# s3prl/s3prl

Measured on AMD Instinct MI355X. Metric: encoder-frames/sec (20 ms stride) HuBERT-base 32x10 s @16 kHz, higher is better.
Workload: dtype f32; 1 GPU; hubert_base random-init, 32x10 s @16 kHz per GPU, one UpstreamExpert.forward per step: all 13 hidden_states (fp32) written; utterances_per_gpu=32, global_batch=32, samples=160000, frames_per_utt=499, parallelism=dp1, lengths=equal, gather=none

## Files before the change

### s3prl_amd/csrc/engine.hip

```cpp
#include "engine_internal.h"

namespace s3e {

thread_local std::string g_err;

long conv_len(const s3enc_config& c, long n, int upto ) {
    for (int i = 0; i < upto; ++i) n = n >= c.conv_kernel[i] ? (n - c.conv_kernel[i]) / c.conv_stride[i] + 1 : 0;
    return n;
}

int valid_frames(const s3enc_config& c, long length, long n_max) {
    const long T = conv_len(c, n_max, c.n_conv);
    if (T <= 0) return 0;
    long v;
    if (c.family == S3ENC_WAV2VEC2 || c.family == S3ENC_DISTILLER || c.family == S3ENC_WAV2VEC) {
        v = conv_len(c, length, c.n_conv);
    } else {
        const long chunk = n_max / T;
        v = (length + chunk - 1) / chunk;
    }
    if (v > T) v = T;
    if (v < 0) v = 0;
    return (int)v;
}
// ... 236 lines not shown
            }
            if (e->x3 || (e->x2_conv_f32_from && i >= e->x2_conv_f32_from)) UP(upload_x3(e->conv[i].w3, t2, C, (long)k * cin));
            if (e->dtype == F32 && !e->x3 && k == 3 && c.conv_stride[i] == 2) {
                std::vector<float> wp((size_t)C * cin);
                for (int co = 0; co < C; ++co)
                    for (int ci = 0; ci < cin; ++ci) wp[(size_t)co * cin + ci] = t2[(long)co * 3 * cin + ci] + t2[(long)co * 3 * cin + 2 * cin + ci];
                UP(upload_f32(e->conv[i].wp, wp));
            }
        }
        if (c.conv_bias) {
            GET(p + ".0.bias", C, t);
            UP(upload_f32(e->conv[i].bias, t));
            e->conv[i].has_bias = true;
        }
        if (c.extractor_layer_norm) {
            GET(p + ".2.1.weight", C, t);
            UP(upload_f32(e->conv[i].lng, t));
            GET(p + ".2.1.bias", C, t);
            UP(upload_f32(e->conv[i].lnb, t));
        } else if (i == 0) {
            GET(p + ".2.weight", C, t);
            UP(upload_f32(e->gn_g, t));
            GET(p + ".2.bias", C, t);
            UP(upload_f32(e->gn_b, t));
        }
    }
    if (!c.no_feature_layer_norm) {
        GET("layer_norm.weight", C, t);
        UP(upload_f32(e->fln_g, t));
        GET("layer_norm.bias", C, t);
        UP(upload_f32(e->fln_b, t));
    }
    GET("post_extract_proj.weight", (long)D * C, t);
    UP(upload_gemm_w(e->proj_w, t, D, C, e->dtype, e->x2));
    e->x2_proj_f32 = e->x2 && !c.no_feature_layer_norm && c.family != S3ENC_DISTILLER && x3_shape_ok(D, C, C);
    if (e->x3 || e->x2_proj_f32) UP(upload_x3(e->proj_w3, t, D, C));
    GET("post_extract_proj.bias", D, t);
    UP(upload_f32(e->proj_b, t));

    const bool conf = c.layer_type == 1;
    if (conf) {
    } else if (c.pos_conv_depth > 1) {
        const int G = c.conv_pos_groups, Dg = D / G;
        int k = c.conv_pos / c.pos_conv_depth;
        k = k < 3 ? 3 : k;
        const bool k16 = e->dtype != F32 || e->x3;
        int kp = k;
        if (k16)
            while ((kp & 1) || ((long)kp * Dg) % 128) ++kp;
        e->pos_k = kp;
        e->pos_pad = k / 2;
        e->pos_ws.resize(c.pos_conv_depth);
        e->pos_bs.resize(c.pos_conv_depth);
        for (int i = 0; i < c.pos_conv_depth; ++i) {
            const std::string p = "encoder.pos_conv." + std::to_string(i) + ".0";
            std::vector<float> w, wp((size_t)D * Dg * kp, 0.f);
            GET(p + ".weight", (long)D * Dg * k, w);
            for (long r = 0; r < (long)D * Dg; ++r)
                for (int j = 0; j < k; ++j) wp[r * kp + j] = w[r * k + j];
            if (e->x3) {
                UP(upload_posconv_x3(e->pos_ws[i], wp, D, G, kp));
            } else {
                pack_posconv(wp, D, G, kp, e->dtype, t2);
                UP(upload_cvt(e->pos_ws[i], t2, e->dtype));
            }
            GET(p + ".bias", D, t);
            UP(upload_f32(e->pos_bs[i], t));
        }
        UP(upload_f32(e->ones, std::vector<float>(D, 1.f)));
        UP(upload_f32(e->zeros, std::vector<float>(D, 0.f)));
    } else {
        const int K = c.conv_pos, G = c.conv_pos_groups, Dg = D / G;
        std::vector<float> g, v;
        GET(enc0 + ".pos_conv.0.weight_g", K, g);
        GET(enc0 + ".pos_conv.0.weight_v", (long)D * Dg * K, v);
        std::vector<double> nrm(K, 0.0);
        for (long i = 0; i < (long)D * Dg; ++i)
            for (int k = 0; k < K; ++k) nrm[k] += (double)v[i * K + k] * v[i * K + k];
        for (int k = 0; k < K; ++k) nrm[k] = (double)g[k] / std::sqrt(nrm[k]);
        for (long i = 0; i < (long)D * Dg; ++i)
            for (int k = 0; k < K; ++k) v[i * K + k] = (float)(v[i * K + k] * nrm[k]);
        int kp = K;
        if (e->dtype != F32 || e->x3)
            while ((kp & 1) || ((long)kp * Dg) % 128) ++kp;
        e->pos_k = kp;
        e->pos_pad = K / 2;
        if (kp != K) {
            std::vector<float> vp((size_t)D * Dg * kp, 0.f);
            for (long r = 0; r < (long)D * Dg; ++r)
                for (int j = 0; j < K; ++j) vp[r * kp + j] = v[r * K + j];
            v.swap(vp);
        }
        pack_posconv(v, D, G, kp, e->dtype, t2);
        UP(upload_cvt(e->pos_w, t2, e->dtype));
        if (e->x3) UP(upload_posconv_x3(e->pos_w3, v, D, G, kp));
        GET(enc0 + ".pos_conv.0.bias", D, t);
        UP(upload_f32(e->pos_b, t));
    }
    if (!multires) {
        GET("encoder.layer_norm.weight", D, t);
        UP(upload_f32(e->eln_g, t));
        GET("encoder.layer_norm.bias", D, t);
        UP(upload_f32(e->eln_b, t));
    }

    const float qscale = (1.0f / std::sqrt((float)(D / H))) * (e->dtype != F32 ? 1.44269504088896340736f : 1.0f);
    e->x2_attn_f32 = e->x2 && !multires && x3_shape_ok(D, D, D);
    auto load_layer = [&](const std::string& p, LayerW& L) -> int {
        std::vector<float> w(3L * D * D), bb(3L * D);
        const char* names[3] = {"q_proj", "k_proj", "v_proj"};
        for (int s = 0; s < 3; ++s) {
            GET(p + ".self_attn." + names[s] + ".weight", (long)D * D, t);
            GET(p + ".self_attn." + names[s] + ".bias", D, t2);
            const float sc = s == 0 ? qscale : 1.f;
            for (long i = 0; i < (long)D * D; ++i) w[(long)s * D * D + i] = t[i] * sc;
            for (int i = 0; i < D; ++i) bb[(long)s * D + i] = t2[i] * sc;
        }
        UPW(L.wqkv, w, 3L * D, D, 2);
        if (e->x3) UP(upload_x3(L.wqkv3, w, 3L * D, D));
        UP(upload_f32(L.bqkv, bb));
        GET(p + ".self_attn.out_proj.weight", (long)D * D, t);
        UP(upload_gemm_w(L.wo, t, D, D, e->dtype, e->x2));
        if (e->x3 || e->x2_attn_f32) UP(upload_x3(L.wo3, t, D, D));
        GET(p + ".self_attn.out_proj.bias", D, t);
        UP(upload_f32(L.bo, t));
        GET(p + ".self_attn_layer_norm.weight", D, t);
        UP(upload_f32(L.ln1g, t));
        GET(p + ".self_attn_layer_norm.bias", D, t);
        UP(upload_f32(L.ln1b, t));
        GET(p + ".fc1.weight", (long)F * D, t);
        UPW(L.w1, t, F, D, 4);
        if (e->x3) UP(upload_x3(L.w13, t, F, D));
        GET(p + ".fc1.bias", F, t);
        UP(upload_f32(L.b1, t));
        GET(p + ".fc2.weight", (long)D * F, t);
        UPW(L.w2, t, D, F, 8);
        if (e->x3) UP(upload_x3(L.w23, t, D, F));
        GET(p + ".fc2.bias", D, t);
        UP(upload_f32(L.b2, t));
        GET(p + ".final_layer_norm.weight", D, t);
        UP(upload_f32(L.ln2g, t));
        GET(p + ".final_layer_norm.bias", D, t);
        UP(upload_f32(L.ln2b, t));
        if (c.rel_pos && c.gru_rel_pos) {
            GET(p + ".self_attn.grep_linear.weight", 8 * 64, t);
            UP(upload_f32(L.grep_w, t));
            GET(p + ".self_attn.grep_linear.bias", 8, t);
            UP(upload_f32(L.grep_b, t));
// ... 798 lines not shown
        e->taps["feat_ln"] = {featT, M * C, proj32 ? (int)F32 : dt};
        if (dbg_stop == 20) return 0;
    }
    const int si_proj = (dist || (conf && c.layer_norm_first)) ? 0 : -1;
    float* xproj = sink.slot32(si_proj) ? sink.slot32(si_proj) : (float*)x32;
    {
        GemmParams g{};
        g.A = featT;
        g.lda = C;
        g.a_bs = T * C;
        g.W = e->proj_w.p;
        g.W_x3 = e->proj_w3.p;
        g.bias = (const float*)e->proj_b.p;
        g.M = (int)T;
        g.N = D;
        g.K = C;
        g.batches = B;
        g.row_limit = d_valid;
        g.out32 = xproj;
        g.out16 = sink.slot16(si_proj);
        g.ldo = D;
        g.o_bs = T * D;
        {
            Prof pr(e, st, "gemm:proj", 2.0 * M * D * C, ((double)M * C + (double)D * C) * es + (double)M * D * 4);
            if (proj32 && dt != F32) {
                if (!gemm_x3_eligible(g)) return fail("post_extract_proj is not a shape of the three-term GEMM (internal)");
                HIP_TRY(launch_gemm(F32, g, st));
            } else {
                HIP_TRY(launch_gemm(dt, wsplit_of(e, g), st));
            }
        }
        e->taps["proj"] = {xproj, M * D, F32};
        if (dbg_stop == 21) return 0;
        HIP_TRY(sink.emit(si_proj, xproj, false));
        HIP_TRY(sink.done(si_proj));
    }
    if (mr) {
        std::vector<const int*> dv(plan.blocks.size(), d_valid);
        for (size_t bi = 1; bi < plan.blocks.size(); ++bi) dv[bi] = (const int*)(d_tbl + (size_t)B * 20) + (bi - 1) * (size_t)B;
        return multires_tail(e, st, B, plan, dv, xproj, out, (long)layer_stride, fo) ? 1 : 0;
    }
    if (conf) {
        ConformerBufs cb{x32, xpc, xT, qkv, attn, tmp1, tmp2, hbuf, cbuf, pbuf};
        return conformer_tail(e, st, sink, B, T, d_valid, xproj, cb);
    }
    float* x_cur;
    void* a16_cur = nullptr;
    {
        const int si0 = si_hidden(0);
        float* pc_out = prel ? (sink.slot32(si0) ? sink.slot32(si0) : other(xproj)) : other(xproj);
        PosConvParams p{};
        p.x = xproj;
        p.w = e->pos_w.p;
        p.bias = (const float*)e->pos_b.p;
        p.out = pc_out;
        p.B = B;
        p.T = (int)T;
        p.D = D;
        p.G = c.conv_pos_groups;
        p.K = e->pos_k;
        p.pad = e->pos_pad;
        auto run_conv = [&](PosConvParams& q) -> hipError_t {
            if (e->x3) return launch_posconv16(3, q, st);
            return dt == F32 ? launch_posconv(q, st) : launch_posconv16(dt, q, st);
        };
        if (c.pos_conv_depth > 1) {
            const float* cur_in = xproj;
            const int gelu_act = (dt != F32 || e->x3) ? 2 : 1;
            for (int i = 0; i < c.pos_conv_depth; ++i) {
                p.x = cur_in;
                p.w = e->pos_ws[i].p;
                p.bias = (const float*)e->pos_bs[i].p;
                p.out = (float*)tmp1;
                p.K = e->pos_k;
                p.pad = e->pos_pad;
                p.plain = 1;
                {
                    Prof pr(e, st, "posconv", 2.0 * M * D * (D / p.G) * (2 * e->pos_pad + 1), (double)M * D * 8);
                    HIP_TRY(run_conv(p));
                }
                Prof pr(e, st, "layernorm:posconv", 0, (double)M * D * 8);
                HIP_TRY(launch_layernorm(F32, (const float*)tmp1, (const float*)e->ones.p, (const float*)e->zeros.p, M, D, gelu_act,
                                         (float*)tmp2, nullptr, st));
                cur_in = (const float*)tmp2;
            }
            Prof pr(e, st, "residual_add", 0, (double)M * D * 12);
            HIP_TRY(launch_add(xproj, (const float*)tmp2, pc_out, M * D, st));
            p.out = pc_out;
        } else {
            Prof pr(e, st, "posconv", 2.0 * M * D * (D / p.G) * c.conv_pos, (double)M * D * 8 + (double)D * (D / p.G) * c.conv_pos * 4);
            if (e->x3) p.w = e->pos_w3.p;
            HIP_TRY(run_conv(p));
        }
        e->taps["posconv"] = {p.out, M * D, F32};
        if (dbg_stop == 22) return 0;
        if (prel) {
            x_cur = pc_out;
            if (sink.mode == 1) HIP_TRY(sink.emit(si0, pc_out));
            HIP_TRY(sink.done(si0));
        } else {
            float* h0 = sink.slot32(si0) ? sink.slot32(si0) : other(pc_out);
            void* h16 = dt == F32 ? nullptr : (sink.slot16(si0) ? sink.slot16(si0) : xT);
            Prof pr(e, st, "layernorm:enc", 0, (double)M * D * (8 + (dt == F32 ? 0 : es)));
            LnGate g0;
            if (gated) {
                g0.gw = (const float*)e->layers[0].grep_w.p;
                g0.gb = (const float*)e->layers[0].grep_b.p;
                g0.ga = (const float*)e->layers[0].grep_a.p;
                g0.gate = (float*)gate;
                g0.T = (int)T;
                g0.H = H;
            }
            HIP_TRY(launch_layernorm(dt, pc_out, (const float*)e->eln_g.p, (const float*)e->eln_b.p, M, D, 0, h0, h16, st,
                                     sink.acc(si0, 2), g0));
            x_cur = h0;
            a16_cur = h16;
            HIP_TRY(sink.done(si0));
        }
    }
    const float* d_table = c.rel_pos ? (const float*)e->rel_table.p : nullptr;
    auto gate_of = [&](int l) {
        LnGate g;
        if (gated && l < NL) {
            const LayerW& w = e->layers[l];
// ... 403 lines not shown
```

### s3prl_amd/csrc/engine_internal.h

```cpp
#pragma once
#include <hip/hip_runtime.h>

#include <algorithm>
#include <cmath>
#include <cstdio>
#include <cstring>
#include <map>
#include <memory>
#include <mutex>
#include <string>
#include <thread>
#include <vector>

#include "../../include/s3enc.h"
#include "kernels.h"

namespace s3e {
using namespace s3;


extern thread_local std::string g_err;

inline int fail(const std::string& msg) {
    g_err = msg;
// ... 98 lines not shown

inline hipError_t upload_f32(DevBuf& d, const std::vector<float>& v) {
    hipError_t e = d.ensure(v.size() * 4 + 16);
    if (e != hipSuccess) return e;
    return hipMemcpy(d.p, v.data(), v.size() * 4, hipMemcpyHostToDevice);
}
template <typename F>
inline void parallel_ranges(long n, long min_per_thread, F&& fn) {
    unsigned nt = std::thread::hardware_concurrency();
    nt = nt < 1 ? 1 : (nt > 16 ? 16 : nt);
    if ((long)nt > n / std::max<long>(1, min_per_thread)) nt = (unsigned)std::max<long>(1, n / std::max<long>(1, min_per_thread));
    if (nt <= 1) {
        fn(0L, n);
        return;
    }
    std::vector<std::thread> th;
    unsigned started = 0;
    try {
        th.reserve(nt);
        for (; started < nt; ++started) th.emplace_back([&fn, n, nt, started]() { fn(n * started / nt, n * (started + 1) / nt); });
    } catch (...) {
    }
    for (unsigned t = started; t < nt; ++t) fn(n * t / nt, n * (t + 1) / nt);
    for (auto& x : th) x.join();
}

inline hipError_t upload_cvt(DevBuf& d, const std::vector<float>& v, int dtype) {
    if (dtype == F32) return upload_f32(d, v);
    std::vector<uint16_t> h(v.size());
    const float* src = v.data();
    uint16_t* dst = h.data();
    if (dtype == BF16)
        parallel_ranges((long)v.size(), 1 << 20, [=](long a, long b) { for (long i = a; i < b; ++i) dst[i] = h_bf16(src[i]); });
    else
        parallel_ranges((long)v.size(), 1 << 20, [=](long a, long b) { for (long i = a; i < b; ++i) dst[i] = h_f16(src[i]); });
    hipError_t e = d.ensure(h.size() * 2 + 16);
    if (e != hipSuccess) return e;
    return hipMemcpy(d.p, h.data(), h.size() * 2, hipMemcpyHostToDevice);
}

inline void pack_posconv(const std::vector<float>& w, int D, int G, int K, int dtype, std::vector<float>& out) {
    const int Dg = D / G;
    out.assign((size_t)G * K * Dg * Dg, 0.f);
    for (int gi = 0; gi < G; ++gi)
        for (int n = 0; n < Dg; ++n)
            for (int ci = 0; ci < Dg; ++ci)
                for (int k = 0; k < K; ++k) {
                    const float x = w[((long)(gi * Dg + n) * Dg + ci) * K + k];
                    if (dtype == F32)
                        out[((((long)gi * K + k) * (Dg / 16) + ci / 16) * Dg + n) * 16 + ((((ci % 16) >> 2) ^ pc_w_swizzle(n)) << 2) + (ci & 3)] = x;
                    else
                        out[(((long)gi * Dg + n) * K + k) * Dg + ci] = x;
                }
}

inline hipError_t upload_f16_hi_lo(DevBuf& d, const std::vector<float>& v, long N, long K) {
    std::vector<uint16_t> h((size_t)N * 2 * K);
    const float* src = v.data();
    uint16_t* dst = h.data();
    parallel_ranges(N, std::max<long>(1, (1 << 19) / std::max<long>(1, K)), [=](long n0, long n1) {
        for (long n = n0; n < n1; ++n)
            for (long k = 0; k < K; ++k) {
                const float w = src[(size_t)n * K + k];
                const uint16_t hi = h_f16(w);
                dst[(size_t)n * 2 * K + k] = hi;
                dst[(size_t)n * 2 * K + K + k] = h_f16(w - h_from16(hi, F16));
            }
    });
    hipError_t e = d.ensure(h.size() * 2 + 16);
    if (e != hipSuccess) return e;
    return hipMemcpy(d.p, h.data(), h.size() * 2, hipMemcpyHostToDevice);
}
inline hipError_t upload_gemm_w(DevBuf& d, const std::vector<float>& v, long N, long K, int dtype, bool x2) {
    return x2 ? upload_f16_hi_lo(d, v, N, K) : upload_cvt(d, v, dtype);
}

inline unsigned mx_e2m1(float x) {
    const unsigned sign = x < 0.f ? 8u : 0u;
    const float a = x < 0.f ? -x : x;
    unsigned c;
    if (a < 0.25f) c = 0; else if (a == 0.25f) c = 0;
    else if (a < 0.75f) c = 1; else if (a == 0.75f) c = 2;
    else if (a < 1.25f) c = 2; else if (a == 1.25f) c = 2;
    else if (a < 1.75f) c = 3; else if (a == 1.75f) c = 4;
    else if (a < 2.5f) c = 4; else if (a == 2.5f) c = 4;
    else if (a < 3.5f) c = 5; else if (a == 3.5f) c = 6;
    else if (a < 5.f) c = 6; else if (a == 5.f) c = 6;
    else c = 7;
    return sign | c;
}
inline void pack_mx4_lo_rows(const float* w, long K, long n0, long n1, uint8_t* data, uint8_t* scales) {
    const long kb = K / 32;
    for (long n = n0; n < n1; ++n)
        for (long b = 0; b < kb; ++b) {
            float lo[32], amax = 0.f;
            for (int i = 0; i < 32; ++i) {
                const float x = w[(size_t)n * K + b * 32 + i];
                lo[i] = x - h_from16(h_f16(x), F16);
                const float a = lo[i] < 0.f ? -lo[i] : lo[i];
                amax = a > amax ? a : amax;
            }
            int ex = -127;
            if (!(amax <= 3.0e38f)) {
                ex = 128;
            } else if (amax > 0.f) {
                ex = (int)ceilf(log2f(amax / 6.f));
// ... 70 lines not shown
struct ConvW {
    DevBuf w, bias, lng, lnb;
    DevBuf w3;
    DevBuf wp;
    bool has_bias = false;
};

struct BlockW {
    std::vector<LayerW> layers;
    DevBuf eln_g, eln_b;
};
struct AdapterConvW {
    DevBuf w, w3;
    DevBuf g, b;
};
struct AdapterW {
    AdapterConvW up, down;
    int kind = 0;
    int up_rate = 1, down_rate = 1;
};

struct W2vW {
    std::vector<DevBuf> ext_w, ext_g, ext_b;
    std::vector<DevBuf> agg_w, agg_bias, agg_g, agg_b;
    std::vector<DevBuf> vq_w, vq_b;
    std::vector<DevBuf> km_w;
    DevBuf km_g, km_b, emb_t;
    DevBuf table;
};

struct ProfRec {
    int kind;
    hipEvent_t a, b;
};

}

using namespace s3e;

struct s3enc_encoder {
    s3enc_config cfg;
    int device = 0;
    int dtype = F32;
    bool x3 = false;
    bool x2 = false;
    int x2_conv_f32_from = 0;
    bool x2_proj_f32 = false;
    bool x2_attn_f32 = false;
    int es = 4;
    std::vector<ConvW> conv;
    DevBuf gn_g, gn_b;
    DevBuf fln_g, fln_b, proj_w, proj_b, pos_w, pos_b, eln_g, eln_b;
    DevBuf proj_w3, pos_w3;
    std::vector<LayerW> layers;
    std::vector<ConformerLayerW> cf_layers;
    DevBuf rope_tab, pe_tab;
    int rope_T = 0, pe_T = 0;
    DevBuf rel_table;
    int rel_R = 0;
    std::vector<DevBuf> pos_ws, pos_bs;
    int pos_k = 0, pos_pad = 0;
    DevBuf ones, zeros;
    DevBuf head_w1, head_b1, head_w2, head_b2, head_w13, head_w23;
    DevBuf wsum_part;
    std::vector<BlockW> mr_blocks;
    std::vector<AdapterW> mr_adapters;
    DevBuf ws_mr;
    std::unique_ptr<W2vW> w2v;
    s3enc_wav2vec_config w2v_cfg = {};
    float* aux_codewords = nullptr;
    long long* aux_codeids = nullptr;

    std::map<const void*, std::unique_ptr<MxImage>> mx_images;

    Tuning tun;
    bool has_tuning = false;

    DevBuf ws;
    DevBuf small;
    void* pinned = nullptr;
    static constexpr int RING = 4;
    size_t slot_bytes = 0;
    hipEvent_t slot_ev[RING] = {};
    int slot_next = 0;

    std::vector<hipEvent_t> layer_events;

    static constexpr int STATUS_RING = 8;
    DevBuf status_dev;
    int* status_host = nullptr;
    hipEvent_t status_ev[STATUS_RING] = {};
    bool status_busy[STATUS_RING] = {};
    int status_next = 0;
    int status_sticky = 0;
    int status_collect(bool wait) {
        int running = 0;
        for (int k = 0; k < STATUS_RING; ++k) {
            const int i = (status_next + k) % STATUS_RING;
            if (!status_busy[i]) continue;
            const hipError_t q = wait ? hipEventSynchronize(status_ev[i]) : hipEventQuery(status_ev[i]);
            if (q == hipErrorNotReady) {
                (void)hipGetLastError();
                ++running;
                continue;
            }
            status_busy[i] = false;
            if (q == hipSuccess) status_sticky |= ((volatile int*)status_host)[i];
        }
        return running;
    }

    int prof = 0;
    std::vector<std::string> kinds;
// ... 153 lines not shown
```

### s3prl_amd/csrc/kernels.h

```cpp
#pragma once
#include <cstring>
#include <vector>

#include "common.h"

namespace s3 {
int device_cus();

template <auto Kern>
inline hipError_t ensure_dynamic_lds(int bytes) {
    static int granted[64] = {};
    int dev = 0;
    hipError_t e = hipGetDevice(&dev);
    if (e != hipSuccess) return e;
    if (dev >= 0 && dev < 64 && granted[dev] >= bytes) return hipSuccess;
    e = hipFuncSetAttribute((const void*)Kern, hipFuncAttributeMaxDynamicSharedMemorySize, bytes);
    if (e == hipSuccess && dev >= 0 && dev < 64) granted[dev] = bytes;
    return e;
}

struct Tuning {
    int gemm_variant = 3;
    int gemm_lds_pad = 0;
    int gemm32_big = 1;
    int gemm_x3_tile = 1;
    int gemm16_big = 3;
    int gemm16_pp = 0;
    int gemm16_mx = 14;
    int reserve_cus = 0;
    int gemm16_rows = 1;
    int attn_lds_pad = 0;
    int attn_persist = 0;
    int conv0_nt = 1;
    int conv_f22 = 1;
    int conv0_fast = 1;
    int ws_inplace = 1;
    int gelu32 = 1;
    int x3_pack_cache = 0;
    int fp16x2_conv1_f32 = 0;
    int ln_rows = 1;
    int ln_preload = 1;
    int ln1_fold = 1;
    int gn_lag_one_block = 1;
    int forward_chain = 1;
    int comm_self_p2p = 0;
};
extern Tuning g_tuning;
extern thread_local const Tuning* t_tuning;
inline const Tuning& tuning() { return t_tuning ? *t_tuning : g_tuning; }
struct TuningScope {
    const Tuning* prev;
    explicit TuningScope(const Tuning* t) : prev(t_tuning) { if (t) t_tuning = t; }
    ~TuningScope() { t_tuning = prev; }
};
int tuning_set(Tuning& t, const char* key, int value, const char** err);

extern thread_local int* t_status;
struct StatusScope {
    int* prev;
    explicit StatusScope(int* p) : prev(t_status) { t_status = p; }
    ~StatusScope() { t_status = prev; }
};

struct GemmParams {
    const void* A;
    long lda, a_bs;
    const void* W;
    const void* W_x3 = nullptr;
    const float* bias;
    int M, N, K, batches;
    int act;
    const float* residual;
    const int* row_limit;
    const float2* res_ln_stats = nullptr;
    const float* res_ln_g = nullptr;
    const float* res_ln_b = nullptr;
    float* out32;
    void* out16;
    long ldo, o_bs;
    int variant = -1;
    long ldw = 0;
    int wsplit = 0;
    const void* W4 = nullptr;
    const void* W4s = nullptr;
    int mxw = 0;
};
bool gemm16_mx_eligible(int dtype, const GemmParams& p);
// ... 59 lines not shown
    float w = 0.f;
    int mode = 0;
    int norm = 0;
    int init = 0;
};
struct LnGate {
    const float* gw = nullptr;
    const float* gb = nullptr;
    const float* ga = nullptr;
    float* gate = nullptr;
    int T = 0, H = 0;
};
hipError_t launch_layernorm(int dtype, const float* x, const float* gamma, const float* beta, long rows, int C, int act,
                            float* out32, void* out16, hipStream_t s, const LnAcc& fa = LnAcc(), const LnGate& gt = LnGate(),
                            float2* stats_out = nullptr);
hipError_t launch_emit_state(int dtype, const float* x, long rows, int C, void* out16, const LnAcc& fa, hipStream_t s);
hipError_t launch_add(const float* a, const float* b, float* out, long n, hipStream_t s);

struct AttnParams {
    const void* qkv;
    void* out;
    const int* valid;
    int B, T, H;
    const float* bias_table;
    int table_R = 0;
    const float* gate;
    int out_f32 = 0;
    int probe = 0;
    const float* rel_P = nullptr;
    const float* rel_qadd = nullptr;
};
hipError_t launch_attention(int dtype, const AttnParams& p, hipStream_t s);
hipError_t launch_wavlm_gate(const float* x, const float* grep_w , const float* grep_b ,
                             const float* grep_a , int B, int T, int H, float* gate, hipStream_t s);

struct ConformerConvParams {
    const float* x;
    const float* taps;
    const float* shift;
    float* out;
    int B, T, D, K;
};
hipError_t launch_conformer_conv(const ConformerConvParams& p, hipStream_t s);
hipError_t launch_rope(const float* x, const float* table, long rows, int T, int D, float* out, hipStream_t s);

struct PosConvParams {
    const float* x;
    const void* w;
    const float* bias;
    float* out;
    int B, T, D, G, K;
    int pad = -1;
    int plain = 0;
};
hipError_t launch_posconv(const PosConvParams& p, hipStream_t s);
__host__ __device__ inline int pc_w_swizzle(int co) { return ((co & 15) >> 3) << 1; }
hipError_t launch_posconv16(int dtype, const PosConvParams& p, hipStream_t s);

struct PadCopyParams {
    const float* a;
    long a_bs;
    const float* b;
    long b_bs;
    int B, rows, D;
    int lead, total;
    const int* zero_from;
    float* out32;
    void* out16;
};
hipError_t launch_pad_copy(int dtype, const PadCopyParams& p, hipStream_t s);
constexpr int GS_BLOCKS = 64;
hipError_t launch_group1_stats(const float* x, long bs, long count, int B, double* partial , hipStream_t s);
struct AdapterApplyParams {
    const float* conv;
    long conv_bs;
    const double* partial;
    double count;
    const float* gamma;
    const float* beta;
    const float* r1;
    long r1_bs;
    int r1_mul, r1_div;
    const float* r2;
    long r2_bs;
    int r2_mul, r2_div;
    float scale;
    int B, rows, D;
    int lead, total;
    const int* zero_from;
    float* out32;
    void* out16;
    int fast_gelu;
};
hipError_t launch_adapter_apply(int dtype, const AdapterApplyParams& p, hipStream_t s);
hipError_t launch_emit_upsampled(int dtype, const float* x, long x_bs, int factor, int B, int rows_out, int D, float* out32,
                                 void* out16, hipStream_t s);

hipError_t launch_emit_upsampled_acc(const float* x, long x_bs, int factor, int B, int rows_out, int D, const LnAcc& fa,
                                     hipStream_t s);

struct Gn1ApplyParams {
    const float* x;
    long x_bs;
    const double* partial;
    double count;
    const float* gamma;
// ... 50 lines not shown
```

### s3prl_amd/csrc/multires.hip

```cpp
#include "engine_internal.h"

namespace s3e {

long mr_adapter_frames(int k, long T, int up, int down, int kind) {
    long n = T;
    if (kind != 1) n = std::min<long>((long)up * T + k - 1, (long)up * T);
    if (kind != 2) {
        const long ld = (n + 2 * ((k - 1) / 2) - k) / down + 1;
        const long n2 = std::min(ld, (n + down - 1) / down);
        n = kind == 0 ? std::min(n2, ((long)up * T + down - 1) / down) : n2;
    }
    return n;
}

void mr_plan(const s3enc_config& c, long T0, MrPlan& plan) {
    const int R = c.mr_pairs + 1, k = c.mr_kernel;
    long ds[S3ENC_MAX_RES], lcm = 1;
    ds[0] = 1;
    for (int i = 0; i < c.n_conv; ++i) ds[0] *= c.conv_stride[i];
    for (int i = 0; i < R - 1; ++i) ds[i + 1] = ds[i] * c.mr_ratios[2 * i + 1] / c.mr_ratios[2 * i];
    for (int i = 0; i < R; ++i) {
        long a = lcm, b = ds[i];
        while (b) {
            const long r = a % b;
// ... 80 lines not shown
        attn = wb.take((size_t)Mc * D * es);
        hbuf = wb.take((size_t)Mc * F * es);
        for (int i = 0; i < R - 1; ++i) res[i] = (float*)wb.take((size_t)B * plan.blocks[i].T * D * 4);
        for (int i = 0; i < 2; ++i) {
            pad32[i] = (float*)wb.take((size_t)B * Pc * D * 4);
            if (dt != F32) pad16[i] = wb.take((size_t)B * Pc * D * 2);
        }
        convout = (float*)wb.take((size_t)B * Lc * D * 4);
        gpart = (double*)wb.take((size_t)B * GS_BLOCKS * 2 * 8);
        if (!pass) HIP_TRY(e->ws_mr.ensure_on_stream(wb.off + 4096, st));
    }

    int si = 0;
    bool first_term = true;
    auto emit = [&](const float* x, long T, int factor) -> int {
        if (fo.featurize) {
            if (fo.w[si] != 0.f) {
                LnAcc fa;
                fa.acc = (float*)out;
                fa.w = fo.w[si];
                fa.mode = 1;
                fa.norm = fo.feat_norm;
                fa.init = first_term;
                first_term = false;
                Prof pr(e, st, "emit_state", 0, (double)B * plan.T_out * D * (4.0 / factor + 8));
                HIP_TRY(launch_emit_upsampled_acc(x, T * D, factor, B, (int)plan.T_out, D, fa, st));
            }
            ++si;
            return 0;
        }
        float* o32 = out16 ? nullptr : (float*)out + (long)si * layer_stride;
        void* o16 = out16 ? (void*)((u16*)out + (long)si * layer_stride) : nullptr;
        {
            Prof pr(e, st, "emit_state", 0, (double)B * plan.T_out * D * (4.0 / factor + (out16 ? 2 : 4)));
            HIP_TRY(launch_emit_upsampled(out16 ? dt : (int)F32, x, T * D, factor, B, (int)plan.T_out, D, o32, o16, st));
        }
        if (si < (int)e->layer_events.size()) HIP_TRY(hipEventRecord(e->layer_events[si], st));
        ++si;
        return 0;
    };

    auto run_block = [&](int bi, float* x, float* y_out) -> int {
        BlockW& bw = e->mr_blocks[bi];
        const MrBlockPlan& bp = plan.blocks[bi];
        const long T = bp.T, M = (long)B * T;
        const double gM = (double)M;
        const int NLb = (int)bw.layers.size();
        float* cur = x;
        auto pick = [&](const float* busy) { return busy == hA ? hB : hA; };
        if (bi == 0) {
            PosConvParams p{};
            p.x = x;
            p.w = e->x3 ? e->pos_w3.p : e->pos_w.p;
            p.bias = (const float*)e->pos_b.p;
            p.out = hA;
            p.B = B;
            p.T = (int)T;
            p.D = D;
            p.G = c.conv_pos_groups;
            p.K = e->pos_k;
            p.pad = e->pos_pad;
            Prof pr(e, st, "posconv", 2.0 * gM * D * (D / p.G) * c.conv_pos, gM * D * 8 + (double)D * (D / p.G) * p.K * 4);
            HIP_TRY(e->x3 ? launch_posconv16(3, p, st) : (dt == F32 ? launch_posconv(p, st) : launch_posconv16(dt, p, st)));
            cur = hA;
        }
        if (!prel) {
            float* h0 = pick(cur);
            Prof pr(e, st, "layernorm:enc", 0, gM * D * (8 + (dt == F32 ? 0 : es)));
            HIP_TRY(launch_layernorm(dt, cur, (const float*)bw.eln_g.p, (const float*)bw.eln_b.p, M, D, 0, h0,
                                     dt == F32 ? nullptr : xT, st));
            cur = h0;
        }
        if (emit(cur, T, bp.factor)) return 1;
        for (int l = 0; l < NLb; ++l) {
            LayerW& Lw = bw.layers[l];
            const bool lastl = l == NLb - 1;
            const void* a_in;
            if (prel) {
                Prof pr(e, st, "layernorm:ln1", 0, gM * D * (4 + es));
                HIP_TRY(launch_layernorm(dt, cur, (const float*)Lw.ln1g.p, (const float*)Lw.ln1b.p, M, D, 0,
                                         dt == F32 ? (float*)xT : nullptr, dt == F32 ? nullptr : xT, st));
                a_in = xT;
            } else {
                a_in = dt == F32 ? (const void*)cur : (const void*)xT;
            }
            {
                GemmParams g{};
                g.A = a_in;
                g.lda = D;
                g.W = Lw.wqkv.p;
                g.W_x3 = Lw.wqkv3.p;
                g.bias = (const float*)Lw.bqkv.p;
                g.M = (int)M;
                g.N = 3 * D;
                g.K = D;
                g.batches = 1;
                g.ldo = 3 * D;
                if (dt == F32) g.out32 = (float*)qkv; else g.out16 = qkv;
                Prof pr(e, st, "gemm:qkv", 2.0 * gM * 3 * D * D, (gM * D + 3.0 * D * D + gM * 3 * D) * es);
                HIP_TRY(launch_gemm(dt, wsplit_of(e, g), st));
            }
            {
                AttnParams a{};
                a.qkv = qkv;
                a.out = attn;
                a.valid = d_valid[bi];
// ... 250 lines not shown
```

### s3prl_amd/csrc/ops.hip

```cpp
#include "engine_internal.h"

namespace s3 {
Tuning g_tuning;
thread_local const Tuning* t_tuning = nullptr;
thread_local int* t_status = nullptr;

int tuning_set(Tuning& t, const char* key, int value, const char** err) {
    struct Key {
        const char* name;
        int Tuning::*field;
        int lo, hi;
    };
    static const Key keys[] = {
        {"gemm_variant", &Tuning::gemm_variant, 0, 63},      {"gemm_lds_pad", &Tuning::gemm_lds_pad, 0, 120 * 1024},
        {"gemm32_big", &Tuning::gemm32_big, 0, 5},           {"gemm_x3_tile", &Tuning::gemm_x3_tile, 0, 5},
        {"gemm16_big", &Tuning::gemm16_big, 0, 10},          {"gemm16_rows", &Tuning::gemm16_rows, 0, 1},
        {"attn_lds_pad", &Tuning::attn_lds_pad, 0, 48 * 1024}, {"conv0_nt", &Tuning::conv0_nt, 0, 1},
        {"ws_inplace", &Tuning::ws_inplace, 0, 1},           {"gemm16_pp", &Tuning::gemm16_pp, 0, 3},
        {"gemm16_mx", &Tuning::gemm16_mx, 0, 31},            {"reserve_cus", &Tuning::reserve_cus, 0, 128},
        {"x3_pack_cache", &Tuning::x3_pack_cache, 0, 1},     {"gelu32", &Tuning::gelu32, 0, 1},
        {"comm_self_p2p", &Tuning::comm_self_p2p, 0, 1},     {"attn_persist", &Tuning::attn_persist, 0, 1},
        {"fp16x2_conv1_f32", &Tuning::fp16x2_conv1_f32, 0, 1}, {"gn_lag_one_block", &Tuning::gn_lag_one_block, 0, 1},
        {"ln_rows", &Tuning::ln_rows, 1, 2},                 {"ln1_fold", &Tuning::ln1_fold, 0, 1},
        {"ln_preload", &Tuning::ln_preload, 0, 1},           {"forward_chain", &Tuning::forward_chain, 0, 1},
        {"conv0_fast", &Tuning::conv0_fast, 0, 1},           {"conv_f22", &Tuning::conv_f22, 0, 1},
    };
    static thread_local char msg[160];
    if (!key) {
        *err = "s3enc_set_tuning: null key";
        return 1;
    }
    for (const Key& k : keys)
        if (!strcmp(key, k.name)) {
            if (value < k.lo || value > k.hi) {
                snprintf(msg, sizeof(msg), "%s must be %d..%d", k.name, k.lo, k.hi);
                *err = msg;
                return 1;
            }
            t.*(k.field) = value;
            return 0;
        }
    snprintf(msg, sizeof(msg), "s3enc_set_tuning: unknown key '%s'", key);
    *err = msg;
    return 1;
}
}

extern "C" {

int s3enc_set_tuning(const char* key, int32_t value) {
    const char* err = nullptr;
    if (tuning_set(g_tuning, key, value, &err)) return fail(err);
    return 0;
}
int s3enc_set_handle_tuning(s3enc_handle h, const char* key, int32_t value) {
    if (!h) return fail("null handle");
    if (!h->has_tuning) {
        h->tun = g_tuning;
        h->has_tuning = true;
    }
    const char* err = nullptr;
    if (tuning_set(h->tun, key, value, &err)) return fail(err);
    return 0;
}

int s3enc_op_gemm(int32_t dtype, const void* A, int64_t lda, int64_t a_batch_stride, const void* W, const float* bias, int32_t M,
                  int32_t N, int32_t K, int32_t batches, int32_t act, const float* residual, const int32_t* row_limit,
                  float* out32, void* out16, int64_t ldo, int64_t o_batch_stride, void* stream) {
    GemmParams g{};
    g.A = A;
    g.lda = lda;
    g.a_bs = a_batch_stride;
    g.W = W;
    g.bias = bias;
    g.M = M;
    g.N = N;
    g.K = K;
    g.batches = batches;
// ... 239 lines not shown
    hipStream_t st = (hipStream_t)stream;
    const size_t tbl = (size_t)B * 16, part = stats_partial_elems(B, nm);
    DevBuf buf;
    Bump sz(nullptr);
    sz.take(tbl);
    sz.take((size_t)B * sizeof(float2));
    sz.take((size_t)B * C * sizeof(float2));
    sz.take(part * 8);
    HIP_TRY(buf.ensure(sz.off + 256));
    Bump bb(buf.p);
    char* d_tbl = (char*)bb.take(tbl);
    float2* d_norm = (float2*)bb.take((size_t)B * sizeof(float2));
    float2* d_gn = (float2*)bb.take((size_t)B * C * sizeof(float2));
    double* d_part = (double*)bb.take(part * 8);
    std::vector<char> host(tbl);
    memcpy(host.data(), wavs, (size_t)B * 8);
    for (int b = 0; b < B; ++b) ((long*)(host.data() + (size_t)B * 8))[b] = (long)lengths[b];
    HIP_TRY(hipMemcpy(d_tbl, host.data(), tbl, hipMemcpyHostToDevice));
    WavTable wt{(const float* const*)d_tbl, (const long*)(d_tbl + (size_t)B * 8), B, nm};
    HIP_TRY(launch_wav_norm_stats(wt, normalize, d_part, d_norm, st));
    if (gn_gamma) HIP_TRY(launch_gn_stats(wt, d_norm, w0, gn_gamma, gn_beta, C, k0, stride, L0, d_part, nullptr, d_gn, st));
    Conv0Params p{};
    p.wav = wt;
    p.norm = d_norm;
    p.w0 = w0;
    p.bias = bias;
    p.gn = gn_gamma ? d_gn : nullptr;
    p.ln_g = ln_gamma;
    p.ln_b = ln_beta;
    p.C = C;
    p.k0 = k0;
    p.s0 = stride;
    p.L0 = L0;
    p.out = out;
    HIP_TRY(launch_conv0(dtype, p, st));
    HIP_TRY(hipStreamSynchronize(st));
    return 0;
}

int s3enc_op_wavlm_gate(const float* x, const float* grep_w, const float* grep_b, const float* grep_a, int32_t B, int32_t T,
                        int32_t H, float* gate, void* stream) {
    if (!x || !grep_w || !grep_b || !grep_a || !gate) return fail("s3enc_op_wavlm_gate: null argument");
    if (B <= 0 || T <= 0 || H <= 0) return fail("s3enc_op_wavlm_gate: bad shape");
    HIP_TRY(launch_wavlm_gate(x, grep_w, grep_b, grep_a, B, T, H, gate, (hipStream_t)stream));
    return 0;
}

int s3enc_op_posconv(int32_t dtype, const float* x, const float* w_host, const float* bias, int32_t B, int32_t T, int32_t D,
                     int32_t G, int32_t K, float* out, void* stream) {
    if (!x || !w_host || !bias || !out) return fail("s3enc_op_posconv: null argument");
    if (G <= 0 || D % G) return fail("s3enc_op_posconv: D must be a multiple of groups");
    const int Dg = D / G;
    std::vector<float> w(w_host, w_host + (size_t)D * Dg * K), packed;
    DevBuf dw;
    if (dtype == 3) {
        HIP_TRY(upload_posconv_x3(dw, w, D, G, K));
    } else {
        pack_posconv(w, D, G, K, dtype, packed);
        HIP_TRY(upload_cvt(dw, packed, dtype));
    }
    PosConvParams p{};
    p.x = x;
    p.w = dw.p;
    p.bias = bias;
    p.out = out;
    p.B = B;
    p.T = T;
    p.D = D;
    p.G = G;
    p.K = K;
    HIP_TRY(dtype == F32 ? launch_posconv(p, (hipStream_t)stream) : launch_posconv16(dtype, p, (hipStream_t)stream));
    HIP_TRY(hipStreamSynchronize((hipStream_t)stream));
    return 0;
}

int s3enc_weighted_sum(const float* hs, int64_t layer_stride, int32_t L, const float* w, int32_t normalize, int64_t rows, int32_t D,
                       float* out, void* stream) {
    if (!hs || !w || !out) return fail("s3enc_weighted_sum: null argument");
    if (L <= 0 || L > S3_WS_MAX_LAYERS) return fail("s3enc_weighted_sum: 1..32 layers");
    if (D <= 0 || (D & 3) || D > 2048) return fail("s3enc_weighted_sum: D must be a multiple of 4, <= 2048");
    HIP_TRY(launch_weighted_sum(hs, layer_stride, L, w, normalize, rows, D, out, (hipStream_t)stream));
    return 0;
}

int64_t s3enc_weighted_sum_backward_scratch(int64_t rows, int32_t L) {
    return rows > 0 && L > 0 ? (int64_t)weighted_sum_bwd_blocks(rows) * L : 0;
}

int s3enc_weighted_sum_backward(const float* hs, int64_t layer_stride, int32_t L, int32_t normalize, int64_t rows, int32_t D,
                                const float* grad_out, float* grad_w, double* scratch, void* stream) {
    if (!hs || !grad_out || !grad_w || !scratch) return fail("s3enc_weighted_sum_backward: null argument");
    if (L <= 0 || L > S3_WS_MAX_LAYERS) return fail("s3enc_weighted_sum_backward: 1..32 layers");
    if (D <= 0 || (D & 3) || D > 2048) return fail("s3enc_weighted_sum_backward: D must be a multiple of 4, <= 2048");
    if (rows <= 0) return fail("s3enc_weighted_sum_backward: no rows");
    HIP_TRY(launch_weighted_sum_bwd(hs, layer_stride, L, normalize, rows, D, grad_out, scratch, grad_w, (hipStream_t)stream));
    return 0;
}

static FbankParams fbank_params(const s3enc_fbank_config* c) {
    FbankParams f;
    f.sample_rate = c->sample_rate;
    f.num_mel_bins = c->num_mel_bins;
    f.frame_length_ms = c->frame_length_ms;
    f.frame_shift_ms = c->frame_shift_ms;
    f.preemph = c->preemphasis;
    f.delta_order = c->delta_order;
    f.delta_win = c->delta_win_length;
    f.use_cmvn = c->use_cmvn;
    f.cmvn_eps = c->cmvn_eps;
    return f;
}

int s3enc_fbank_num_frames(const s3enc_fbank_config* cfg, int64_t n_samples, int32_t* frames) {
    if (!cfg || !frames) return fail("s3enc_fbank_num_frames: null argument");
    *frames = (int32_t)fbank_num_frames(n_samples, fbank_params(cfg));
    return 0;
// ... 25 lines not shown
```

### s3prl_amd/csrc/posconv.hip

```cpp
#include "kernels.h"

namespace s3 {
namespace {

constexpr int PC_TM = 128;
constexpr int PC_FT = 2;

struct PcWork {
    int b, g, tile;
    bool live;
};
__device__ __forceinline__ PcWork pc_work(const PosConvParams& p, int ntiles) {
    PcWork w;
    const int wg = blockIdx.x;
    if (p.G & 7) {
        w.tile = wg % ntiles;
        const int r = wg / ntiles;
        w.g = r % p.G;
        w.b = r / p.G;
        w.live = w.b < p.B;
        return w;
    }
    const int per = ntiles * p.B, xcd = wg & 7, local = wg >> 3;
    w.g = xcd + 8 * (local / per);
// ... 61 lines not shown

    const float* xrow = xs + (wave * (16 * PC_FT) + l15) * RS + 4 * kk;
    for (int j = 0; j < K; ++j) {
        if (j + 1 < K) wload(j + 1);
        const float* wb = wl + (j & 1) * WSZ + l15 * 16 + 4 * (kk ^ pc_w_swizzle(l15));
        const float* xa = xrow + j * RS;
#pragma unroll
        for (int cc = 0; cc < NCC; ++cc) {
            float4 a[PC_FT];
#pragma unroll
            for (int f = 0; f < PC_FT; ++f) a[f] = *(const float4*)(xa + f * 16 * RS + 16 * cc);
#pragma unroll
            for (int n = 0; n < NT; ++n) {
                const float4 w = *(const float4*)(wb + (cc * DG + n * 16) * 16);
#pragma unroll
                for (int f = 0; f < PC_FT; ++f) {
                    acc[f][n] = __builtin_amdgcn_mfma_f32_16x16x4f32(a[f].x, w.x, acc[f][n], 0, 0, 0);
                    acc[f][n] = __builtin_amdgcn_mfma_f32_16x16x4f32(a[f].y, w.y, acc[f][n], 0, 0, 0);
                    acc[f][n] = __builtin_amdgcn_mfma_f32_16x16x4f32(a[f].z, w.z, acc[f][n], 0, 0, 0);
                    acc[f][n] = __builtin_amdgcn_mfma_f32_16x16x4f32(a[f].w, w.w, acc[f][n], 0, 0, 0);
                }
            }
        }
        if (j + 1 < K) wstore((j + 1) & 1);
        __syncthreads();
    }

#pragma unroll
    for (int f = 0; f < PC_FT; ++f)
#pragma unroll
        for (int n = 0; n < NT; ++n) {
            const int c = g * DG + n * 16 + l15;
            const float bias = p.bias[c];
#pragma unroll
            for (int r = 0; r < 4; ++r) {
                const int t = t0 + wave * (16 * PC_FT) + 16 * f + 4 * kk + r;
                if (t < p.T) {
                    const long o = ((long)b * p.T + t) * p.D + c;
                    p.out[o] = p.plain ? acc[f][n][r] + bias : p.x[o] + gelu_erf(acc[f][n][r] + bias);
                }
            }
        }
}

template <int DG>
hipError_t pc_launch(const PosConvParams& p, hipStream_t s) {
    const int rows = PC_TM + p.K - 1;
    const size_t lds = (size_t)(((rows * (DG + 8) + 3) & ~3) + 2 * DG * DG) * sizeof(float);
    hipError_t e = ensure_dynamic_lds<posconv_kernel<DG>>((int)lds);
    if (e != hipSuccess) return e;
    dim3 grid((unsigned)(((p.T + PC_TM - 1) / PC_TM) * p.G * p.B));
    hipLaunchKernelGGL(posconv_kernel<DG>, grid, dim3(256), lds, s, p);
    return hipGetLastError();
}


constexpr int P16_TM = 256;
constexpr int P16_KC = 128;

template <typename T> struct Mma16x16;
template <> struct Mma16x16<bf16_tag> {
    static __device__ __forceinline__ f32x4 run(const uint4& a, const uint4& b, const f32x4& c) {
        return __builtin_amdgcn_mfma_f32_16x16x32_bf16(__builtin_bit_cast(bf16x8, a), __builtin_bit_cast(bf16x8, b), c, 0, 0, 0);
    }
};
template <> struct Mma16x16<f16_tag> {
    static __device__ __forceinline__ f32x4 run(const uint4& a, const uint4& b, const f32x4& c) {
        return __builtin_amdgcn_mfma_f32_16x16x32_f16(__builtin_bit_cast(f16x8, a), __builtin_bit_cast(f16x8, b), c, 0, 0, 0);
    }
};

template <typename T, int DG, bool X3>
__global__ __launch_bounds__(256) void posconv16_kernel(PosConvParams p) {
    constexpr int NT = DG / 16;
    constexpr int CH = DG / 8;
    constexpr int NLW = DG * 16 / 256;
    constexpr int WBUF = DG * 256;
    constexpr int NS = X3 ? 2 : 1;
    constexpr int TMF = X3 ? 128 : P16_TM;
    constexpr int MT = TMF / 64;
    extern __shared__ __attribute__((aligned(16))) char lds16[];
    const int K = p.K;
    const int ROWS = (TMF + K - 1 + 15) & ~15;
    const size_t WIN = (size_t)CH * ROWS * 16;
    char* win = lds16;
    char* wl = lds16 + NS * WIN;

    const PcWork wk = pc_work(p, (p.T + TMF - 1) / TMF);
    if (!wk.live) return;
    const int b = wk.b, g = wk.g;
    const int t0 = wk.tile * TMF;
    const int tid = threadIdx.x, lane = tid & 63, wave = tid >> 6;
    const int l15 = lane & 15, kgrp = lane >> 4;
    const int pad = p.pad >= 0 ? p.pad : K / 2;
    const long Ktot = (long)K * DG;

    const char* wg = (const char*)p.w + (long)g * DG * Ktot * 2;
    const long plane_bytes = (long)p.G * DG * Ktot * 2;
    u32x4 wreg[NS][NLW];
#define P16_WLOAD(kc_)                                                                                        \
    _Pragma("unroll") for (int s_ = 0; s_ < NS; ++s_) _Pragma("unroll") for (int i_ = 0; i_ < NLW; ++i_) {  \
        const int e_ = tid + 256 * i_, n_ = e_ >> 4, c_ = e_ & 15;                                          \
        wreg[s_][i_] = *(const u32x4*)(wg + s_ * plane_bytes + ((long)n_ * Ktot + (long)(kc_) * P16_KC + c_ * 8) * 2); \
    }
#define P16_WSTORE(buf_)                                                                                      \
    _Pragma("unroll") for (int s_ = 0; s_ < NS; ++s_) _Pragma("unroll") for (int i_ = 0; i_ < NLW; ++i_) {  \
// ... 74 lines not shown
#pragma unroll
        for (int m = 0; m < MT; ++m)
#pragma unroll
            for (int r = 0; r < 4; ++r) {
                const int t = t0 + wave * (TMF / 4) + m * 16 + 4 * kgrp + r;
                if (t < p.T) {
                    const long o = ((long)b * p.T + t) * p.D + c;
                    const float y = acc[m][n][r] + bias;
                    p.out[o] = p.plain ? y : p.x[o] + gelu_fast(y);
                }
            }
    }
}

template <typename T, int DG, bool X3>
hipError_t pc16_launch(const PosConvParams& p, hipStream_t s) {
    constexpr int NS = X3 ? 2 : 1, TMF = X3 ? 128 : P16_TM;
    const int ROWS = (TMF + p.K - 1 + 15) & ~15;
    const size_t lds = (size_t)NS * (DG / 8) * ROWS * 16 + (size_t)NS * 2 * DG * 256;
    if (lds > 160 * 1024) return hipErrorInvalidValue;
    hipError_t e = ensure_dynamic_lds<posconv16_kernel<T, DG, X3>>((int)lds);
    if (e != hipSuccess) return e;
    dim3 grid((unsigned)(((p.T + TMF - 1) / TMF) * p.G * p.B));
    hipLaunchKernelGGL((posconv16_kernel<T, DG, X3>), grid, dim3(256), lds, s, p);
    return hipGetLastError();
}

template <typename T, bool X3 = false>
hipError_t pc16_dispatch(const PosConvParams& p, int dg, hipStream_t s) {
    switch (dg) {
        case 32: return pc16_launch<T, 32, X3>(p, s);
        case 48: return pc16_launch<T, 48, X3>(p, s);
        case 64: return pc16_launch<T, 64, X3>(p, s);
    }
    return hipErrorInvalidValue;
}

}

hipError_t launch_posconv16(int dtype, const PosConvParams& p, hipStream_t s) {
    if (p.B <= 0 || p.T <= 0) return hipSuccess;
    const int dg = p.D / p.G;
    if (dg * p.G != p.D || (p.K & 1) || ((long)p.K * dg) % P16_KC) return hipErrorInvalidValue;
    if (dtype == BF16) return pc16_dispatch<bf16_tag>(p, dg, s);
    if (dtype == F16) return pc16_dispatch<f16_tag>(p, dg, s);
    if (dtype == 3) return pc16_dispatch<bf16_tag, true>(p, dg, s);
    return hipErrorInvalidValue;
}

hipError_t launch_posconv(const PosConvParams& p, hipStream_t s) {
    if (p.B <= 0 || p.T <= 0) return hipSuccess;
    const int dg = p.D / p.G;
    if (dg * p.G != p.D) return hipErrorInvalidValue;
    switch (dg) {
        case 32: return pc_launch<32>(p, s);
        case 48: return pc_launch<48>(p, s);
        case 64: return pc_launch<64>(p, s);
    }
    return hipErrorInvalidValue;
}

}
```

Baseline: 459,700 frames/s.

## Add Winograd-style F(2,2) fp32 positional conv kernel using precomputed tap-pair weight sums

Adds a new fp32 grouped positional-convolution kernel that produces two output frames per tap pair, using precomputed sums of adjacent kernel taps so each pair of taps needs three matrix products instead of four. The input is split into even and odd rows in LDS, and weight stages are double-buffered through registers with MFMA 16x16x4 f32. Host code packs and uploads the summed-weight tensors for even K in fp32 mode and passes them to the kernel, which is selected by a new tuning flag that is on by default. This cuts roughly a quarter of the conv FLOPs, at the cost of extra LDS, extra weight memory, and slightly different fp32 rounding.

```diff
diff --git a/s3prl_amd/csrc/engine.hip b/s3prl_amd/csrc/engine.hip
--- a/s3prl_amd/csrc/engine.hip
+++ b/s3prl_amd/csrc/engine.hip
@@ -312,6 +312,7 @@
         e->pos_pad = k / 2;
         e->pos_ws.resize(c.pos_conv_depth);
         e->pos_bs.resize(c.pos_conv_depth);
+        e->pos_wsums.resize(c.pos_conv_depth);
         for (int i = 0; i < c.pos_conv_depth; ++i) {
             const std::string p = "encoder.pos_conv." + std::to_string(i) + ".0";
             std::vector<float> w, wp((size_t)D * Dg * kp, 0.f);
@@ -323,6 +324,7 @@
             } else {
                 pack_posconv(wp, D, G, kp, e->dtype, t2);
                 UP(upload_cvt(e->pos_ws[i], t2, e->dtype));
+                if (e->dtype == F32 && !(kp & 1)) UP(upload_posconv_sum(e->pos_wsums[i], wp, D, G, kp));
             }
             GET(p + ".bias", D, t);
             UP(upload_f32(e->pos_bs[i], t));
@@ -354,6 +356,7 @@
         pack_posconv(v, D, G, kp, e->dtype, t2);
         UP(upload_cvt(e->pos_w, t2, e->dtype));
         if (e->x3) UP(upload_posconv_x3(e->pos_w3, v, D, G, kp));
+        if (e->dtype == F32 && !e->x3 && !(kp & 1)) UP(upload_posconv_sum(e->pos_wsum, v, D, G, kp));
         GET(enc0 + ".pos_conv.0.bias", D, t);
         UP(upload_f32(e->pos_b, t));
     }
@@ -1258,6 +1261,7 @@
         PosConvParams p{};
         p.x = xproj;
         p.w = e->pos_w.p;
+        p.ws = (const float*)e->pos_wsum.p;
         p.bias = (const float*)e->pos_b.p;
         p.out = pc_out;
         p.B = B;
@@ -1276,6 +1280,7 @@
             for (int i = 0; i < c.pos_conv_depth; ++i) {
                 p.x = cur_in;
                 p.w = e->pos_ws[i].p;
+                p.ws = (const float*)e->pos_wsums[i].p;
                 p.bias = (const float*)e->pos_bs[i].p;
                 p.out = (float*)tmp1;
                 p.K = e->pos_k;
diff --git a/s3prl_amd/csrc/engine_internal.h b/s3prl_amd/csrc/engine_internal.h
--- a/s3prl_amd/csrc/engine_internal.h
+++ b/s3prl_amd/csrc/engine_internal.h
@@ -174,6 +174,23 @@
                     else
                         out[(((long)gi * Dg + n) * K + k) * Dg + ci] = x;
                 }
+}
+
+inline void pack_posconv_sum(const std::vector<float>& w, int D, int G, int K, std::vector<float>& out) {
+    const int Dg = D / G, KH = K / 2;
+    out.assign((size_t)G * KH * Dg * Dg, 0.f);
+    for (int gi = 0; gi < G; ++gi)
+        for (int n = 0; n < Dg; ++n)
+            for (int ci = 0; ci < Dg; ++ci)
+                for (int j = 0; j < KH; ++j) {
+                    const float* t = &w[((long)(gi * Dg + n) * Dg + ci) * K + 2 * j];
+                    out[((((long)gi * KH + j) * (Dg / 16) + ci / 16) * Dg + n) * 16 + ((((ci % 16) >> 2) ^ pc_w_swizzle(n)) << 2) + (ci & 3)] = t[0] + t[1];
+                }
+}
+inline hipError_t upload_posconv_sum(DevBuf& d, const std::vector<float>& w, int D, int G, int K) {
+    std::vector<float> ws;
+    pack_posconv_sum(w, D, G, K, ws);
+    return upload_f32(d, ws);
 }
 
 inline hipError_t upload_f16_hi_lo(DevBuf& d, const std::vector<float>& v, long N, long K) {
@@ -350,6 +367,7 @@
     DevBuf gn_g, gn_b;
     DevBuf fln_g, fln_b, proj_w, proj_b, pos_w, pos_b, eln_g, eln_b;
     DevBuf proj_w3, pos_w3;
+    DevBuf pos_wsum;
     std::vector<LayerW> layers;
     std::vector<ConformerLayerW> cf_layers;
     DevBuf rope_tab, pe_tab;
@@ -357,6 +375,7 @@
     DevBuf rel_table;
     int rel_R = 0;
     std::vector<DevBuf> pos_ws, pos_bs;
+    std::vector<DevBuf> pos_wsums;
     int pos_k = 0, pos_pad = 0;
     DevBuf ones, zeros;
     DevBuf head_w1, head_b1, head_w2, head_b2, head_w13, head_w23;
diff --git a/s3prl_amd/csrc/kernels.h b/s3prl_amd/csrc/kernels.h
--- a/s3prl_amd/csrc/kernels.h
+++ b/s3prl_amd/csrc/kernels.h
@@ -33,6 +33,7 @@
     int attn_persist = 0;
     int conv0_nt = 1;
     int conv_f22 = 1;
+    int posconv_f22 = 1;
     int conv0_fast = 1;
     int ws_inplace = 1;
     int gelu32 = 1;
@@ -198,6 +199,7 @@
     int B, T, D, G, K;
     int pad = -1;
     int plain = 0;
+    const float* ws = nullptr;
 };
 hipError_t launch_posconv(const PosConvParams& p, hipStream_t s);
 __host__ __device__ inline int pc_w_swizzle(int co) { return ((co & 15) >> 3) << 1; }
diff --git a/s3prl_amd/csrc/multires.hip b/s3prl_amd/csrc/multires.hip
--- a/s3prl_amd/csrc/multires.hip
+++ b/s3prl_amd/csrc/multires.hip
@@ -156,6 +156,7 @@
             PosConvParams p{};
             p.x = x;
             p.w = e->x3 ? e->pos_w3.p : e->pos_w.p;
+            p.ws = (const float*)e->pos_wsum.p;
             p.bias = (const float*)e->pos_b.p;
             p.out = hA;
             p.B = B;
diff --git a/s3prl_amd/csrc/ops.hip b/s3prl_amd/csrc/ops.hip
--- a/s3prl_amd/csrc/ops.hip
+++ b/s3prl_amd/csrc/ops.hip
@@ -24,6 +24,7 @@
         {"ln_rows", &Tuning::ln_rows, 1, 2},                 {"ln1_fold", &Tuning::ln1_fold, 0, 1},
         {"ln_preload", &Tuning::ln_preload, 0, 1},           {"forward_chain", &Tuning::forward_chain, 0, 1},
         {"conv0_fast", &Tuning::conv0_fast, 0, 1},           {"conv_f22", &Tuning::conv_f22, 0, 1},
+        {"posconv_f22", &Tuning::posconv_f22, 0, 1},
     };
     static thread_local char msg[160];
     if (!key) {
@@ -369,7 +370,8 @@
     if (G <= 0 || D % G) return fail("s3enc_op_posconv: D must be a multiple of groups");
     const int Dg = D / G;
     std::vector<float> w(w_host, w_host + (size_t)D * Dg * K), packed;
-    DevBuf dw;
+    DevBuf dw, dws;
+    if (dtype == F32 && K >= 2 && !(K & 1)) HIP_TRY(upload_posconv_sum(dws, w, D, G, K));
     if (dtype == 3) {
         HIP_TRY(upload_posconv_x3(dw, w, D, G, K));
     } else {
@@ -379,6 +381,7 @@
     PosConvParams p{};
     p.x = x;
     p.w = dw.p;
+    p.ws = (const float*)dws.p;
     p.bias = bias;
     p.out = out;
     p.B = B;
diff --git a/s3prl_amd/csrc/posconv.hip b/s3prl_amd/csrc/posconv.hip
--- a/s3prl_amd/csrc/posconv.hip
+++ b/s3prl_amd/csrc/posconv.hip
@@ -137,6 +137,167 @@
     dim3 grid((unsigned)(((p.T + PC_TM - 1) / PC_TM) * p.G * p.B));
     hipLaunchKernelGGL(posconv_kernel<DG>, grid, dim3(256), lds, s, p);
     return hipGetLastError();
+}
+
+constexpr int PF_TMP = 128;
+constexpr int PF_NTH = 512;
+constexpr int PF_FB = 6;
+template <int DG> struct PfCfg {
+    static constexpr int CH = DG == 48 ? 3 : 2;
+    static constexpr int STG = 3 * CH * DG * 16;
+    static constexpr size_t lds_bytes(int K) { return ((size_t)(2 * (PF_TMP + K / 2)) * (DG + 8) + 2 * STG) * sizeof(float); }
+};
+
+template <int DG>
+__global__ __launch_bounds__(PF_NTH) void posconv_f22_kernel(PosConvParams p) {
+    constexpr int NT = DG / 16;
+    constexpr int NCC = DG / 16;
+    constexpr int CH = PfCfg<DG>::CH, NSG = NCC / CH, STG = PfCfg<DG>::STG;
+    constexpr int RS = DG + 8;
+    constexpr int PV = CH * DG * 4;
+    constexpr int NWV = (3 * PV + PF_NTH - 1) / PF_NTH;
+    static_assert(NCC % CH == 0, "a stage holds whole chunks");
+    extern __shared__ __attribute__((aligned(16))) float lds[];
+    const int K = p.K, KH = K >> 1;
+    const int NE = PF_TMP + KH;
+    float* xe = lds;
+    float* xo = lds + NE * RS;
+    float* wl = lds + 2 * NE * RS;
+
+    const PcWork wk = pc_work(p, (p.T + 2 * PF_TMP - 1) / (2 * PF_TMP));
+    if (!wk.live) return;
+    const int b = wk.b, g = wk.g;
+    const int t0 = wk.tile * (2 * PF_TMP);
+    const int tid = threadIdx.x, lane = tid & 63, wave = tid >> 6;
+    const int l15 = lane & 15, kk = lane >> 4;
+    const int pad = p.pad >= 0 ? p.pad : K / 2;
+
+    const f32x4* wg = (const f32x4*)((const float*)p.w + (long)g * K * DG * DG);
+    const f32x4* wsg = (const f32x4*)(p.ws + (long)g * KH * DG * DG);
+    f32x4 wreg[NWV];
+    auto wload = [&](int s) {
+        const int j = s / NSG, sg = s % NSG;
+#pragma unroll
+        for (int i = 0; i < NWV; ++i) {
+            const int e = tid + PF_NTH * i;
+            if (e < 3 * PV) {
+                const int r = e / PV, q = e % PV;
+                wreg[i] = r < 2 ? wg[((long)(2 * j + r) * NCC + sg * CH) * (DG * 4) + q] : wsg[((long)j * NCC + sg * CH) * (DG * 4) + q];
+            }
+        }
+    };
+    auto wstore = [&](int buf) {
+#pragma unroll
+        for (int i = 0; i < NWV; ++i) {
+            const int e = tid + PF_NTH * i;
+            if (e < 3 * PV) *(f32x4*)(wl + buf * STG + 4 * e) = wreg[i];
+        }
+    };
+    wload(0);
+
+    const float* xg = p.x + (long)b * p.T * p.D + g * DG;
+    const int nfill = 2 * NE * (DG / 4);
+    for (int base = tid; base < nfill; base += PF_NTH * PF_FB) {
+        float4 v[PF_FB];
+#pragma unroll
+        for (int i = 0; i < PF_FB; ++i) {
+            const int idx = base + PF_NTH * i;
+            const int rr = idx / (DG / 4), c4 = idx % (DG / 4);
+            const int ts = t0 + rr - pad;
+            v[i] = make_float4(0.f, 0.f, 0.f, 0.f);
+            if (idx < nfill && ts >= 0 && ts < p.T) v[i] = *(const float4*)(xg + (long)ts * p.D + 4 * c4);
+        }
+#pragma unroll
+        for (int i = 0; i < PF_FB; ++i) {
+            const int idx = base + PF_NTH * i;
+            const int rr = idx / (DG / 4), c4 = idx % (DG / 4);
+            if (idx < nfill) *(float4*)(((rr & 1) ? xo : xe) + (rr >> 1) * RS + 4 * c4) = v[i];
+        }
+    }
+    wstore(0);
+    __syncthreads();
+
+    f32x4 acc_e[NT], acc_o[NT], acc_p[NT];
+#pragma unroll
+    for (int n = 0; n < NT; ++n) acc_e[n] = acc_o[n] = acc_p[n] = (f32x4){0.f, 0.f, 0.f, 0.f};
+
+    const int roff = (wave * 16 + l15) * RS + 4 * kk;
+    const float* erow = xe + roff;
+    const float* orow = xo + roff;
+    f32x4 ea[NCC];
+#pragma unroll
+    for (int cc = 0; cc < NCC; ++cc) ea[cc] = *(const f32x4*)(erow + 16 * cc);
+
+    const int ns = KH * NSG;
+    for (int j = 0; j < KH; ++j) {
+#pragma unroll
+        for (int sg = 0; sg < NSG; ++sg) {
+            const int s = j * NSG + sg;
+            if (s + 1 < ns) wload(s + 1);
+            const float* wb = wl + (s & 1) * STG + l15 * 16 + 4 * (kk ^ pc_w_swizzle(l15));
+#pragma unroll
+            for (int c = 0; c < CH; ++c) {
+                const int cc = sg * CH + c;
+                const f32x4 xb = *(const f32x4*)(orow + j * RS + 16 * cc);
+                const f32x4 xc = *(const f32x4*)(erow + (j + 1) * RS + 16 * cc);
+                const f32x4 d0 = ea[cc] - xb, d1 = xc - xb;
+                ea[cc] = xc;
+                f32x4 w0[NT], w1[NT], w2[NT];
+#pragma unroll
+                for (int n = 0; n < NT; ++n) {
+                    w0[n] = *(const f32x4*)(wb + ((0 * CH + c) * DG + n * 16) * 16);
+                    w1[n] = *(const f32x4*)(wb + ((1 * CH + c) * DG + n * 16) * 16);
+                    w2[n] = *(const f32x4*)(wb + ((2 * CH + c) * DG + n * 16) * 16);
+                }
+#pragma unroll
+                for (int i = 0; i < 4; ++i)
+#pragma unroll
+                    for (int n = 0; n < NT; ++n) {
+                        acc_e[n] = __builtin_amdgcn_mfma_f32_16x16x4f32(d0[i], w0[n][i], acc_e[n], 0, 0, 0);
+                        acc_o[n] = __builtin_amdgcn_mfma_f32_16x16x4f32(d1[i], w1[n][i], acc_o[n], 0, 0, 0);
+                        acc_p[n] = __builtin_amdgcn_mfma_f32_16x16x4f32(xb[i], w2[n][i], acc_p[n], 0, 0, 0);
+                    }
+                if (c == 0 && s + 1 < ns) wstore((s + 1) & 1);
+            }
+            __syncthreads();
+        }
+    }
+
+#pragma unroll
+    for (int n = 0; n < NT; ++n) {
+        const int c = g * DG + n * 16 + l15;
+        const float bias = p.bias[c];
+#pragma unroll
+        for (int r = 0; r < 4; ++r)
+#pragma unroll
+            for (int q = 0; q < 2; ++q) {
+                const int fr = 2 * (wave * 16 + 4 * kk + r) + q, rr = fr + pad;
+                const float xr = ((rr & 1) ? xo : xe)[(rr >> 1) * RS + n * 16 + l15];
+                const float y = (q ? acc_o[n][r] : acc_e[n][r]) + acc_p[n][r] + bias;
+                if (t0 + fr < p.T) p.out[((long)b * p.T + t0 + fr) * p.D + c] = p.plain ? y : xr + gelu_erf(y);
+            }
+    }
+}
+
+template <int DG>
+hipError_t pf_launch(const PosConvParams& p, hipStream_t s) {
+    const size_t lds = PfCfg<DG>::lds_bytes(p.K);
+    hipError_t e = ensure_dynamic_lds<posconv_f22_kernel<DG>>((int)lds);
+    if (e != hipSuccess) return e;
+    dim3 grid((unsigned)(((p.T + 2 * PF_TMP - 1) / (2 * PF_TMP)) * p.G * p.B));
+    hipLaunchKernelGGL(posconv_f22_kernel<DG>, grid, dim3(PF_NTH), lds, s, p);
+    return hipGetLastError();
+}
+
+bool pf_eligible(const PosConvParams& p, int dg) {
+    if (!tuning().posconv_f22 || !p.ws || p.K < 2 || (p.K & 1) || p.pad < -1 || p.pad > p.K) return false;
+    constexpr size_t cap = 160 * 1024;
+    switch (dg) {
+        case 32: return PfCfg<32>::lds_bytes(p.K) <= cap;
+        case 48: return PfCfg<48>::lds_bytes(p.K) <= cap;
+        case 64: return PfCfg<64>::lds_bytes(p.K) <= cap;
+    }
+    return false;
 }
 
 
@@ -317,6 +478,11 @@
     if (p.B <= 0 || p.T <= 0) return hipSuccess;
     const int dg = p.D / p.G;
     if (dg * p.G != p.D) return hipErrorInvalidValue;
+    if (pf_eligible(p, dg)) switch (dg) {
+            case 32: return pf_launch<32>(p, s);
+            case 48: return pf_launch<48>(p, s);
+            case 64: return pf_launch<64>(p, s);
+        }
     switch (dg) {
         case 32: return pc_launch<32>(p, s);
         case 48: return pc_launch<48>(p, s);
```

Measured after the change: 464,000 frames/s (median of 6 runs). Within noise of the previous version (+0.9%).
